# hku-mars/Voxel-SLAM

Hardware: AMD Instinct MI355X
Metric: BA iterations/sec (10-frame window, 100k pts/scan) (higher is better)
Workload: dtype f64; 1 GPU; cfg2: W=10, 100000 pts/scan, 50000 voxels per GPU, nnz=500000; global_voxels=50000, parallelism=voxel-shard x1, ranks_seen=1, collectives_per_lm_step=0, allreduce_doubles=0, lm_steps_accepted=2028, lm_steps_rejected=0

## Files before the change

### voxel-slam_amd/csrc/vxba_solve4.hpp

```cpp
#pragma once

typedef double s4v2 __attribute__((ext_vector_type(2)));

constexpr int S4_WAVES = 4;
constexpr int S4_THREADS = 64 * S4_WAVES;
constexpr int S4_ROW = 6;
constexpr int S4_BLK = 64 * S4_ROW + 6;
constexpr int S4_GSLOT = 64 * S4_ROW;

template <int W>
struct S4 {
  static constexpr int N = 6 * W, M = N - 6, B = W - 1;
  static constexpr int TC = 0;
  static constexpr int G = TC + (B > 0 ? B : 1) * S4_BLK;
  static constexpr int BV = G + (B > 0 ? B : 1) * S4_GSLOT;
  static constexpr int ZV = BV + 64;
  static constexpr int XS = ZV + 64;
  static constexpr int DOUBLES = XS + 64;
};

__device__ __forceinline__ double s4_rcp(double d) {
  const double r = __builtin_amdgcn_rcp(d);
  const double e = fma(-d, r, 1.0);
  const double t = fma(e, e, e);
  const double q = fma(r, t, r);
  return fabs(d) > 1e-300 ? q : 0.0;
}

__device__ __forceinline__ void s4_ldl6(double (&D)[21], double (&inv)[6]) {
#pragma unroll
  for (int p = 0; p < 6; p++) {
    inv[p] = s4_rcp(D[p * (p + 1) / 2 + p]);
    double col[6];
#pragma unroll
    for (int q = p + 1; q < 6; q++) col[q] = D[q * (q + 1) / 2 + p];
#pragma unroll
    for (int q = p + 1; q < 6; q++) {
      const double l = col[q] * inv[p];
#pragma unroll
      for (int r = p + 1; r <= q; r++) D[q * (q + 1) / 2 + r] = fma(-l, col[r], D[q * (q + 1) / 2 + r]);
      D[q * (q + 1) / 2 + p] = l;
    }
  }
}

__device__ __forceinline__ void s4_load_row(const double* p, double (&a)[6]) {
  const s4v2* v = reinterpret_cast<const s4v2*>(p);
  const s4v2 t0 = v[0], t1 = v[1], t2 = v[2];
  a[0] = t0[0]; a[1] = t0[1]; a[2] = t1[0]; a[3] = t1[1]; a[4] = t2[0]; a[5] = t2[1];
}
__device__ __forceinline__ void s4_store_row(double* p, const double (&a)[6]) {
  s4v2* v = reinterpret_cast<s4v2*>(p);
  v[0] = (s4v2){a[0], a[1]};
  v[1] = (s4v2){a[2], a[3]};
  v[2] = (s4v2){a[4], a[5]};
}

template <int W>
__device__ __forceinline__ void s4_apply(const double* lds, int t, int b, int lane, double (&T)[6]) {
  using C = S4<W>;
  double g[6];
  s4_load_row(lds + C::G + t * S4_GSLOT + lane * S4_ROW, g);
  const double* lr = lds + C::TC + t * S4_BLK + (6 * b) * S4_ROW;
#pragma unroll
  for (int c = 0; c < 6; c++) {
    double l[6];
    s4_load_row(lr + c * S4_ROW, l);
#pragma unroll
    for (int p = 0; p < 6; p++) T[c] = fma(-g[p], l[p], T[c]);
  }
}

constexpr int li_rec_len(int W) { return 1 + 12 * W + 6 * W + 36 * W * W; }
constexpr int li_out_len(int W) { return 6 * W + 12 * W + 1; }
template <int W, bool DBG>
__device__ __forceinline__ int lm_solve_body4(LMState* st, int c, double* lds, const double* __restrict__ li_rec = nullptr, double* __restrict__ li_out = nullptr,
                                               unsigned li_seq = 0) {
  using C = S4<W>;
  LMCtl& ctl = st->ctl[c];
  const int loop_done = ctl.done;
  constexpr int n = C::N, M = C::M, B = C::B;
  const int tid = threadIdx.x, lane = tid & 63;
  const int wave = __builtin_amdgcn_readfirstlane(tid >> 6);
  dbg_stamp(DBG && wave == 0, 4000, 0);
  dbg_stamp(DBG && wave == 0, 4000, 1);
  const double u = li_rec ? li_rec[0] : ctl.u;
  const double* __restrict__ li_x = li_rec ? li_rec + 1 : nullptr;
  const double* __restrict__ li_e = li_rec ? li_rec + 1 + 12 * W : nullptr;
  const double* __restrict__ li_E = li_rec ? li_rec + 1 + 18 * W : nullptr;
  const bool row_ok = lane < M;
  const int gi_row = row_ok ? 6 + lane : 0;

  constexpr int NQ = (B + S4_WAVES - 1) / S4_WAVES;
  double a0[NQ > 0 ? NQ : 1][6];
#pragma unroll
  for (int q = 0; q < NQ; q++) {
    const int b = wave + S4_WAVES * q;
    const int bb = b < B ? b : 0;
#pragma unroll
    for (int cc = 0; cc < 6; cc++) {
      const int col = 6 + 6 * bb + cc;
      const double h = st->Hwork[(size_t)col * n + gi_row];
      const double add = (li_E && gi_row >= 6 + 6 * bb) ? li_E[(size_t)col * n + gi_row] : 0.0;
      a0[q][cc] = row_ok ? (((col == gi_row) ? h + u * h : h) + add) : 0.0;
    }
  }
  double hii = 0.0, gi = 0.0, rhs0 = 0.0;
  double xcur[12];
  if (wave == 0) {
    hii = st->Hwork[(size_t)gi_row * n + gi_row];
    gi = st->Jwork[gi_row];
    const int fl = lane < W ? lane : 0;
#pragma unroll
    for (int k = 0; k < 12; k++) xcur[k] = li_x ? li_x[12 * fl + k] : ctl.x[12 * fl + k];
  }
  if (wave == 1 % S4_WAVES) rhs0 = row_ok ? (li_e ? li_e[gi_row] : 0.0) - st->Jwork[gi_row] : 0.0;
  if (loop_done) return 1;
  if (wave < B) s4_store_row(lds + C::TC + wave * S4_BLK + lane * S4_ROW, a0[0]);
  dbg_stamp(DBG && wave == 0, 4000, 2);

  int ap0 = -1, ap1 = -1, ap2 = -1;
  for (int s = 0; s < B; s++) {
    const int owner = s & (S4_WAVES - 1);
    double Ld[21], inv[6], g[6];
    if (wave == owner) {
      const int sq = s >> 2;
      const int ap = sq == 0 ? ap0 : (sq == 1 ? ap1 : ap2);
      double* trow = lds + C::TC + s * S4_BLK + lane * S4_ROW;
      double a[6];
      dbg_stamp(DBG, 4010 + s, 0);
      s4_load_row(trow, a);
      for (int t = ap + 1; t < s; t++) s4_apply<W>(lds, t, s, lane, a);
      if (DBG) { asm volatile("" :: "v"(a[0]), "v"(a[5])); dbg_stamp(true, 4010 + s, 1); }
      s4_store_row(trow, a);
      __builtin_amdgcn_wave_barrier();
      {
        const double* dr = lds + C::TC + s * S4_BLK + (6 * s) * S4_ROW;
        const s4v2 r0 = *reinterpret_cast<const s4v2*>(dr);
        const s4v2 r1 = *reinterpret_cast<const s4v2*>(dr + 6);
        const s4v2 r2a = *reinterpret_cast<const s4v2*>(dr + 12), r2b = *reinterpret_cast<const s4v2*>(dr + 14);
        const s4v2 r3a = *reinterpret_cast<const s4v2*>(dr + 18), r3b = *reinterpret_cast<const s4v2*>(dr + 20);
        const s4v2 r4a = *reinterpret_cast<const s4v2*>(dr + 24), r4b = *reinterpret_cast<const s4v2*>(dr + 26), r4c = *reinterpret_cast<const s4v2*>(dr + 28);
        const s4v2 r5a = *reinterpret_cast<const s4v2*>(dr + 30), r5b = *reinterpret_cast<const s4v2*>(dr + 32), r5c = *reinterpret_cast<const s4v2*>(dr + 34);
        Ld[0] = r0[0];
        Ld[1] = r1[0]; Ld[2] = r1[1];
        Ld[3] = r2a[0]; Ld[4] = r2a[1]; Ld[5] = r2b[0];
        Ld[6] = r3a[0]; Ld[7] = r3a[1]; Ld[8] = r3b[0]; Ld[9] = r3b[1];
        Ld[10] = r4a[0]; Ld[11] = r4a[1]; Ld[12] = r4b[0]; Ld[13] = r4b[1]; Ld[14] = r4c[0];
        Ld[15] = r5a[0]; Ld[16] = r5a[1]; Ld[17] = r5b[0]; Ld[18] = r5b[1]; Ld[19] = r5c[0]; Ld[20] = r5c[1];
      }
      if (DBG) { asm volatile("" :: "v"(Ld[0]), "v"(Ld[20])); dbg_stamp(true, 4010 + s, 2); }
      s4_ldl6(Ld, inv);
      if (DBG) { asm volatile("" :: "v"(inv[5])); dbg_stamp(true, 4010 + s, 3); }
      double l[6];
#pragma unroll
      for (int p = 0; p < 6; p++) {
        double acc = a[p];
#pragma unroll
        for (int q = 0; q < p; q++) acc = fma(-g[q], Ld[p * (p + 1) / 2 + q], acc);
        g[p] = acc;
        l[p] = acc * inv[p];
      }
      s4_store_row(trow, l);
      s4_store_row(lds + C::G + s * S4_GSLOT + lane * S4_ROW, g);
      if (sq == 0) ap0 = s; else if (sq == 1) ap1 = s; else ap2 = s;
      dbg_stamp(DBG, 4010 + s, 4);
    }
    if (s == 0) {
#pragma unroll
      for (int q = 1; q < NQ; q++) {
        const int b = wave + S4_WAVES * q;
        if (b < B) s4_store_row(lds + C::TC + b * S4_BLK + lane * S4_ROW, a0[q]);
      }
      if (wave == 1 % S4_WAVES) lds[C::BV + lane] = rhs0;
    }
    if (s < 9) dbg_stamp(DBG, 4000 + wave, 6 + 2 * s);
    __syncthreads();
    if (s < 9) dbg_stamp(DBG, 4000 + wave, 7 + 2 * s);
    if (wave == owner) {
      double bb[6];
      s4_load_row(lds + C::BV + 6 * s, bb);
      double br = lds[C::BV + lane];
      double z[6];
#pragma unroll
      for (int p = 0; p < 6; p++) {
        double acc = bb[p];
#pragma unroll
        for (int q = 0; q < p; q++) acc = fma(-bb[q], Ld[p * (p + 1) / 2 + q], acc);
        bb[p] = acc;
        z[p] = acc * inv[p];
      }
#pragma unroll
      for (int p = 0; p < 6; p++) br = fma(-g[p], z[p], br);
      const int d = lane - 6 * s;
      double zsel = z[0];
#pragma unroll
      for (int p = 1; p < 6; p++) zsel = (d == p) ? z[p] : zsel;
      if (d >= 0 && d < 6) lds[C::ZV + lane] = zsel;
      else lds[C::BV + lane] = br;
    }
    const bool next_owner = (s + 1 < B) && wave == ((s + 1) & (S4_WAVES - 1));
    if (!next_owner) {
      int budget = 2;
#pragma unroll
      for (int q = 0; q < (B + S4_WAVES - 1) / S4_WAVES; q++) {
        const int b = wave + S4_WAVES * q;
        int ap = q == 0 ? ap0 : (q == 1 ? ap1 : ap2);
        const bool must = b == s + 2;
        if (b > s && b < B && ap < s && (must || budget > 0)) {
          double* trow = lds + C::TC + b * S4_BLK + lane * S4_ROW;
          double T[6];
          s4_load_row(trow, T);
          while (ap < s && (must || budget > 0)) {
            s4_apply<W>(lds, ap + 1, b, lane, T);
            ap++;
            budget--;
          }
          s4_store_row(trow, T);
          if (q == 0) ap0 = ap; else if (q == 1) ap1 = ap; else ap2 = ap;
        }
      }
    }
  }
  __syncthreads();
  dbg_stamp(DBG && wave == 0, 4000, 3);
  if (wave != 0) return 0;

  double x = row_ok ? lds[C::ZV + lane] : 0.0;
  if constexpr (B > 0) {
    const int jb = (row_ok ? lane : 0) / 6, jc = (row_ok ? lane : 0) % 6;
    const double* lcol = lds + C::TC + jb * S4_BLK + jc;
    double Lr[6], Ln[6];
#pragma unroll
    for (int k = 0; k < 6; k++) Lr[k] = lcol[(M - 1 - k) * S4_ROW];
    for (int rb = B - 1; rb >= 0; rb--) {
      if (rb > 0) {
#pragma unroll
        for (int k = 0; k < 6; k++) Ln[k] = lcol[(6 * rb - 1 - k) * S4_ROW];
      }
#pragma unroll
      for (int k = 0; k < 6; k++) {
        const int r = 6 * rb + 5 - k;
        const double xr = readlane_f64(x, r);
        x = (lane < r) ? fma(-Lr[k], xr, x) : x;
      }
#pragma unroll
      for (int k = 0; k < 6; k++) Lr[k] = Ln[k];
    }
  }
  dbg_stamp(DBG, 4000, 4);
  if (row_ok) st->dxi[6 + lane] = x;
  if (lane < 6) st->dxi[lane] = 0.0;
  double* xs = lds + C::XS;
  if (lane < 6) xs[lane] = 0.0;
  if (row_ok) xs[6 + lane] = x;
  __builtin_amdgcn_wave_barrier();
  if (lane < W) {
    double dl[6];
#pragma unroll
    for (int k = 0; k < 6; k++) dl[k] = xs[6 * lane + k];
    double xn[9];
    lm_right_multiply_exp(xcur, dl, xn);
#pragma unroll
    for (int k = 0; k < 9; k++) __hip_atomic_store(&ctl.xt[12 * lane + k], xn[k], __ATOMIC_RELAXED, __HIP_MEMORY_SCOPE_AGENT);
#pragma unroll
    for (int k = 0; k < 3; k++) __hip_atomic_store(&ctl.xt[12 * lane + 9 + k], xcur[9 + k] + dl[3 + k], __ATOMIC_RELAXED, __HIP_MEMORY_SCOPE_AGENT);
    if (li_out) {
#pragma unroll
      for (int k = 0; k < 9; k++) li_out[6 * W + 12 * lane + k] = xn[k];
#pragma unroll
      for (int k = 0; k < 3; k++) li_out[6 * W + 12 * lane + 9 + k] = xcur[9 + k] + dl[3 + k];
    }
  }
  if (li_out) {
    if (row_ok) li_out[6 + lane] = x;
    if (lane < 6) li_out[lane] = 0.0;
    asm volatile("s_waitcnt vmcnt(0)" ::: "memory");
    __builtin_amdgcn_wave_barrier();
    if (lane == 0) li_out[18 * W] = (double)li_seq;
  }
  double part = row_ok ? x * (u * hii * x - gi) : 0.0;
#pragma unroll
  for (int off = 32; off > 0; off >>= 1) part += __shfl_down(part, off);
  if (lane == 0) ctl.q1 = 0.5 * part;
  if (DBG) { asm volatile("s_waitcnt vmcnt(0)" ::: "memory"); dbg_stamp(true, 4000, 5); }
  return 0;
}
```

Before: 21230 iterations/s.

## Replace per-step block barriers with LDS flag-based producer/consumer pipeline in block LDL

Restructures the blocked LDL factorization so wave 0 factors every diagonal block sequentially, while the other waves apply trailing updates and the RHS forward solve asynchronously. Coordination goes through LDS sequence flags with spin-waits instead of a __syncthreads per step. The aim is to remove the barrier on each step's critical path and let wave 0 apply the next block's update itself, using in-register g. The cost is added spin-loop complexity with a timeout error path, the risk of LDS ordering bugs from relying on volatile and compiler fences, and possible load imbalance from pinning all diagonal work to one wave.

```diff
diff --git a/voxel-slam_amd/csrc/vxba_solve4.hpp b/voxel-slam_amd/csrc/vxba_solve4.hpp
--- a/voxel-slam_amd/csrc/vxba_solve4.hpp
+++ b/voxel-slam_amd/csrc/vxba_solve4.hpp
@@ -7,6 +7,9 @@
 constexpr int S4_ROW = 6;
 constexpr int S4_BLK = 64 * S4_ROW + 6;
 constexpr int S4_GSLOT = 64 * S4_ROW;
+constexpr int S4_LDSLOT = 28;
+constexpr int S4_PUB = 0, S4_PUBL = 1, S4_RHS = 2, S4_COL = 4;
+constexpr unsigned S4_SPIN_LIMIT = 1u << 20;
 
 template <int W>
 struct S4 {
@@ -16,7 +19,9 @@
   static constexpr int BV = G + (B > 0 ? B : 1) * S4_GSLOT;
   static constexpr int ZV = BV + 64;
   static constexpr int XS = ZV + 64;
-  static constexpr int DOUBLES = XS + 64;
+  static constexpr int LD = XS + 64;
+  static constexpr int FL = LD + (B > 0 ? B : 1) * S4_LDSLOT;
+  static constexpr int DOUBLES = FL + 16;
 };
 
 __device__ __forceinline__ double s4_rcp(double d) {
@@ -57,10 +62,8 @@
 }
 
 template <int W>
-__device__ __forceinline__ void s4_apply(const double* lds, int t, int b, int lane, double (&T)[6]) {
+__device__ __forceinline__ void s4_apply_g(const double* lds, int t, int b, const double (&g)[6], double (&T)[6]) {
   using C = S4<W>;
-  double g[6];
-  s4_load_row(lds + C::G + t * S4_GSLOT + lane * S4_ROW, g);
   const double* lr = lds + C::TC + t * S4_BLK + (6 * b) * S4_ROW;
 #pragma unroll
   for (int c = 0; c < 6; c++) {
@@ -69,6 +72,51 @@
 #pragma unroll
     for (int p = 0; p < 6; p++) T[c] = fma(-g[p], l[p], T[c]);
   }
+}
+template <int W>
+__device__ __forceinline__ void s4_apply(const double* lds, int t, int b, int lane, double (&T)[6]) {
+  double g[6];
+  s4_load_row(lds + S4<W>::G + t * S4_GSLOT + lane * S4_ROW, g);
+  s4_apply_g<W>(lds, t, b, g, T);
+}
+
+typedef __attribute__((address_space(3))) volatile int s4_seq_t;
+__device__ __forceinline__ int s4_seq_peek(const double* lds, int off, int i) {
+  asm volatile("" ::: "memory");
+  const int v = ((s4_seq_t*)(lds + off))[i];
+  asm volatile("" ::: "memory");
+  return v;
+}
+__device__ __forceinline__ int s4_seq_read(const double* lds, int off, int i) { return __builtin_amdgcn_readfirstlane(s4_seq_peek(lds, off, i)); }
+__device__ __forceinline__ void s4_seq_write(double* lds, int off, int i, int v, int lane) {
+  asm volatile("" ::: "memory");
+  if (lane == 0) ((s4_seq_t*)(lds + off))[i] = v;
+  asm volatile("" ::: "memory");
+}
+
+template <int W>
+__device__ __forceinline__ void s4_rhs(double* lds, int s, int lane, const double (&Ld)[21], const double (&inv)[6], const double (&g)[6]) {
+  using C = S4<W>;
+  double bb[6];
+  s4_load_row(lds + C::BV + 6 * s, bb);
+  double br = lds[C::BV + lane];
+  double z[6];
+#pragma unroll
+  for (int p = 0; p < 6; p++) {
+    double acc = bb[p];
+#pragma unroll
+    for (int q = 0; q < p; q++) acc = fma(-bb[q], Ld[p * (p + 1) / 2 + q], acc);
+    bb[p] = acc;
+    z[p] = acc * inv[p];
+  }
+#pragma unroll
+  for (int p = 0; p < 6; p++) br = fma(-g[p], z[p], br);
+  const int d = lane - 6 * s;
+  double zsel = z[0];
+#pragma unroll
+  for (int p = 1; p < 6; p++) zsel = (d == p) ? z[p] : zsel;
+  if (d >= 0 && d < 6) lds[C::ZV + lane] = zsel;
+  else lds[C::BV + lane] = br;
 }
 
 constexpr int li_rec_len(int W) { return 1 + 12 * W + 6 * W + 36 * W * W; }
@@ -116,23 +164,86 @@
   }
   if (wave == 1 % S4_WAVES) rhs0 = row_ok ? (li_e ? li_e[gi_row] : 0.0) - st->Jwork[gi_row] : 0.0;
   if (loop_done) return 1;
-  if (wave < B) s4_store_row(lds + C::TC + wave * S4_BLK + lane * S4_ROW, a0[0]);
   dbg_stamp(DBG && wave == 0, 4000, 2);
 
-  int ap0 = -1, ap1 = -1, ap2 = -1;
-  for (int s = 0; s < B; s++) {
-    const int owner = s & (S4_WAVES - 1);
-    double Ld[21], inv[6], g[6];
-    if (wave == owner) {
-      const int sq = s >> 2;
-      const int ap = sq == 0 ? ap0 : (sq == 1 ? ap1 : ap2);
-      double* trow = lds + C::TC + s * S4_BLK + lane * S4_ROW;
-      double a[6];
-      dbg_stamp(DBG, 4010 + s, 0);
-      s4_load_row(trow, a);
-      for (int t = ap + 1; t < s; t++) s4_apply<W>(lds, t, s, lane, a);
+  if constexpr (B > 0) {
+    constexpr int NH = B / 3;
+    if (wave != 0) {
+      if (wave < B) s4_store_row(lds + C::TC + wave * S4_BLK + lane * S4_ROW, a0[0]);
+#pragma unroll
+      for (int q = 1; q < NQ; q++) {
+        const int b = wave + S4_WAVES * q;
+        if (b < B) s4_store_row(lds + C::TC + b * S4_BLK + lane * S4_ROW, a0[q]);
+      }
+      if (wave == 1 % S4_WAVES) lds[C::BV + lane] = rhs0;
+      __syncthreads();
+      int ap0 = 0, ap1 = 0, ap2 = 0;
+      int rhs_next = wave == S4_WAVES - 1 ? 0 : B - 1;
+      unsigned spins = 0;
+      for (;;) {
+        const int pub = s4_seq_read(lds, C::FL, S4_PUB);
+        int bsel = -1, apsel = 0;
+        bool open = rhs_next < B - 1;
+#pragma unroll
+        for (int q = 0; q < NH; q++) {
+          const int b = 2 + (wave - 1) + 3 * q;
+          const int ap = q == 0 ? ap0 : (q == 1 ? ap1 : ap2);
+          if (b < B && ap < b - 1) {
+            open = true;
+            if (bsel < 0 && ap < pub) { bsel = b; apsel = ap; }
+          }
+        }
+        if (bsel >= 0) {
+          const int upto = pub < bsel - 1 ? pub : bsel - 1;
+          if (upto <= 9) dbg_stamp(DBG, 4000 + wave, 4 + 2 * upto);
+          double* trow = lds + C::TC + bsel * S4_BLK + lane * S4_ROW;
+          double T[6];
+          s4_load_row(trow, T);
+          for (int t = apsel; t < upto; t++) s4_apply<W>(lds, t, bsel, lane, T);
+          s4_store_row(trow, T);
+          s4_seq_write(lds, C::FL, S4_COL + bsel, upto, lane);
+          if (upto <= 9) dbg_stamp(DBG, 4000 + wave, 5 + 2 * upto);
+          const int q = (bsel - 2) / 3;
+          if (q == 0) ap0 = upto; else if (q == 1) ap1 = upto; else ap2 = upto;
+          spins = 0;
+          continue;
+        }
+        if (rhs_next < B - 1 && s4_seq_read(lds, C::FL, S4_PUBL) > rhs_next) {
+          double Ld[21], inv[6], g[6];
+          const s4v2* v = reinterpret_cast<const s4v2*>(lds + C::LD + rhs_next * S4_LDSLOT);
+          s4v2 t[14];
+#pragma unroll
+          for (int k = 0; k < 14; k++) t[k] = v[k];
+#pragma unroll
+          for (int k = 0; k < 21; k++) Ld[k] = t[k >> 1][k & 1];
+#pragma unroll
+          for (int k = 0; k < 6; k++) inv[k] = t[(21 + k) >> 1][(21 + k) & 1];
+          s4_load_row(lds + C::G + rhs_next * S4_GSLOT + lane * S4_ROW, g);
+          s4_rhs<W>(lds, rhs_next, lane, Ld, inv, g);
+          rhs_next++;
+          s4_seq_write(lds, C::FL, S4_RHS, rhs_next, lane);
+          spins = 0;
+          continue;
+        }
+        if (!open) break;
+        __builtin_amdgcn_s_sleep(1);
+        if (++spins > S4_SPIN_LIMIT) {
+          if (lane == 0) st->error = 3;
+          break;
+        }
+      }
+      return 0;
+    }
+
+    if (lane < 32) ((s4_seq_t*)(lds + C::FL))[lane] = 0;
+    double a[6], Ld[21], inv[6], g[6], l[6];
+#pragma unroll
+    for (int k = 0; k < 6; k++) a[k] = a0[0][k];
+    dbg_stamp(DBG, 4010, 0);
+    for (int s = 0; s < B; s++) {
+      const bool more = s + 1 < B;
       if (DBG) { asm volatile("" :: "v"(a[0]), "v"(a[5])); dbg_stamp(true, 4010 + s, 1); }
-      s4_store_row(trow, a);
+      s4_store_row(lds + C::TC + s * S4_BLK + lane * S4_ROW, a);
       __builtin_amdgcn_wave_barrier();
       {
         const double* dr = lds + C::TC + s * S4_BLK + (6 * s) * S4_ROW;
@@ -152,7 +263,12 @@
       if (DBG) { asm volatile("" :: "v"(Ld[0]), "v"(Ld[20])); dbg_stamp(true, 4010 + s, 2); }
       s4_ldl6(Ld, inv);
       if (DBG) { asm volatile("" :: "v"(inv[5])); dbg_stamp(true, 4010 + s, 3); }
-      double l[6];
+      double T[6];
+      int seen_v = 0;
+      if (more && s > 0) {
+        seen_v = s4_seq_peek(lds, C::FL, S4_COL + s + 1);
+        s4_load_row(lds + C::TC + (s + 1) * S4_BLK + lane * S4_ROW, T);
+      }
 #pragma unroll
       for (int p = 0; p < 6; p++) {
         double acc = a[p];
@@ -161,70 +277,62 @@
         g[p] = acc;
         l[p] = acc * inv[p];
       }
-      s4_store_row(trow, l);
+      s4_store_row(lds + C::TC + s * S4_BLK + lane * S4_ROW, l);
       s4_store_row(lds + C::G + s * S4_GSLOT + lane * S4_ROW, g);
-      if (sq == 0) ap0 = s; else if (sq == 1) ap1 = s; else ap2 = s;
+      s4_seq_write(lds, C::FL, S4_PUB, s + 1, lane);
       dbg_stamp(DBG, 4010 + s, 4);
-    }
-    if (s == 0) {
-#pragma unroll
-      for (int q = 1; q < NQ; q++) {
-        const int b = wave + S4_WAVES * q;
-        if (b < B) s4_store_row(lds + C::TC + b * S4_BLK + lane * S4_ROW, a0[q]);
-      }
-      if (wave == 1 % S4_WAVES) lds[C::BV + lane] = rhs0;
-    }
-    if (s < 9) dbg_stamp(DBG, 4000 + wave, 6 + 2 * s);
-    __syncthreads();
-    if (s < 9) dbg_stamp(DBG, 4000 + wave, 7 + 2 * s);
-    if (wave == owner) {
-      double bb[6];
-      s4_load_row(lds + C::BV + 6 * s, bb);
-      double br = lds[C::BV + lane];
-      double z[6];
-#pragma unroll
-      for (int p = 0; p < 6; p++) {
-        double acc = bb[p];
-#pragma unroll
-        for (int q = 0; q < p; q++) acc = fma(-bb[q], Ld[p * (p + 1) / 2 + q], acc);
-        bb[p] = acc;
-        z[p] = acc * inv[p];
-      }
-#pragma unroll
-      for (int p = 0; p < 6; p++) br = fma(-g[p], z[p], br);
-      const int d = lane - 6 * s;
-      double zsel = z[0];
-#pragma unroll
-      for (int p = 1; p < 6; p++) zsel = (d == p) ? z[p] : zsel;
-      if (d >= 0 && d < 6) lds[C::ZV + lane] = zsel;
-      else lds[C::BV + lane] = br;
-    }
-    const bool next_owner = (s + 1 < B) && wave == ((s + 1) & (S4_WAVES - 1));
-    if (!next_owner) {
-      int budget = 2;
-#pragma unroll
-      for (int q = 0; q < (B + S4_WAVES - 1) / S4_WAVES; q++) {
-        const int b = wave + S4_WAVES * q;
-        int ap = q == 0 ? ap0 : (q == 1 ? ap1 : ap2);
-        const bool must = b == s + 2;
-        if (b > s && b < B && ap < s && (must || budget > 0)) {
-          double* trow = lds + C::TC + b * S4_BLK + lane * S4_ROW;
-          double T[6];
-          s4_load_row(trow, T);
-          while (ap < s && (must || budget > 0)) {
-            s4_apply<W>(lds, ap + 1, b, lane, T);
-            ap++;
-            budget--;
+      if (s == 0) {
+#pragma unroll
+        for (int q = 1; q < NQ; q++) {
+          const int b = S4_WAVES * q;
+          if (b < B) s4_store_row(lds + C::TC + b * S4_BLK + lane * S4_ROW, a0[q]);
+        }
+        __syncthreads();
+      }
+      if (more) {
+        if (s < 9) dbg_stamp(DBG, 4000, 6 + 2 * s);
+        if (s == 0 || __builtin_amdgcn_readfirstlane(seen_v) < s) {
+          unsigned spins = 0;
+          while (s4_seq_read(lds, C::FL, S4_COL + s + 1) < s) {
+            if (++spins > S4_SPIN_LIMIT) {
+              if (lane == 0) st->error = 3;
+              break;
+            }
           }
-          s4_store_row(trow, T);
-          if (q == 0) ap0 = ap; else if (q == 1) ap1 = ap; else ap2 = ap;
-        }
-      }
-    }
-  }
-  __syncthreads();
-  dbg_stamp(DBG && wave == 0, 4000, 3);
-  if (wave != 0) return 0;
+          s4_load_row(lds + C::TC + (s + 1) * S4_BLK + lane * S4_ROW, T);
+        }
+        if (s < 9) dbg_stamp(DBG, 4000, 7 + 2 * s);
+        dbg_stamp(DBG, 4010 + s + 1, 0);
+        s4_apply_g<W>(lds, s, s + 1, g, T);
+#pragma unroll
+        for (int cc = 0; cc < 6; cc++) a[cc] = T[cc];
+        if (lane == 0) {
+          s4v2* v = reinterpret_cast<s4v2*>(lds + C::LD + s * S4_LDSLOT);
+#pragma unroll
+          for (int k = 0; k < 10; k++) v[k] = (s4v2){Ld[2 * k], Ld[2 * k + 1]};
+          v[10] = (s4v2){Ld[20], inv[0]};
+          v[11] = (s4v2){inv[1], inv[2]};
+          v[12] = (s4v2){inv[3], inv[4]};
+          v[13] = (s4v2){inv[5], 0.0};
+        }
+        s4_seq_write(lds, C::FL, S4_PUBL, s + 1, lane);
+      }
+    }
+    if (B > 1) {
+      unsigned spins = 0;
+      while (s4_seq_read(lds, C::FL, S4_RHS) < B - 1) {
+        if (++spins > S4_SPIN_LIMIT) {
+          if (lane == 0) st->error = 3;
+          break;
+        }
+      }
+    }
+    s4_rhs<W>(lds, B - 1, lane, Ld, inv, g);
+    __builtin_amdgcn_wave_barrier();
+  } else {
+    if (wave != 0) return 0;
+  }
+  dbg_stamp(DBG, 4000, 3);
 
   double x = row_ok ? lds[C::ZV + lane] : 0.0;
   if constexpr (B > 0) {
```

Result: slower. 20840 iterations/s (-1.8%).
